# Improbable-AI/walk-these-ways

Hardware: AMD Instinct MI355X
Metric: env-steps/sec (sim+PPO) (higher is better)
Workload: dtype f32

## Files before the change

### include/go1ppo.h

```cpp
#ifndef GO1PPO_H
#define GO1PPO_H
#include <stdint.h>

#ifdef __cplusplus
extern "C" {
#endif

#define GO1PPO_ABI_VERSION 3
#define GO1PPO_MAX_ACTIONS 32

int go1ppo_elu_fwd(void* y, int64_t rows, int cols, int ld, const void* lat, int lat_ld, int npv, const void* wz,
                   int wz_ld, int lat_cols, void* stream);

int go1ppo_elu_bwd(const void* d, int ld_d, const void* h, int ld_h, int64_t rows, int cols, float* bias_grad, void* out,
                   int ld_out, void* stream);

typedef struct {
  const void* mean;
  const void* value;
  const float* std;
  int32_t head_ld, num_actions;
  int64_t rows;
  const int64_t* idx;
  const float* actions;
// ... 71 lines not shown
int go1ppo_store_step(const float* rewards, const uint8_t* dones, const uint8_t* time_outs, const int32_t* env_bins,
                      const float* values, float gamma, int64_t n, float* rewards_out, uint8_t* dones_out,
                      float* env_bins_out, void* stream);

int go1ppo_gae(const float* rewards, const uint8_t* dones, const float* values, const float* last_values, int T, int64_t N,
               float gamma, float lam, float* returns, float* advantages, double* stats, void* stream);

int go1ppo_normalize(float* adv, int64_t n, const double* stats, void* stream);


int go1ppo_ring_snapshot(const float* hist, int64_t ld_hist, int64_t N, int H, int no, void* ring, void* stream);

int go1ppo_ring_step(const float* obs, const float* priv, void* ring_dst, const void* ring_window, int64_t N, int H, int no,
                     int npv, int Kp, void* X, float* obs_store, float* priv_store, void* stream);

int go1ppo_ring_gather(const void* ring, const float* priv_store, const int64_t* idx, int64_t rows, int64_t N, int H, int no,
                       int npv, int Kp, void* X, void* stream);


int go1ppo_opt_partials(void);

int go1ppo_opt_prestep(const float* g, int64_t n, float gscale, float* partial, float* step, float* lr, const float* kl,
                       float kl_scale, float desired_kl, float lr_min, float lr_max, void* stream);

typedef struct {
  int64_t begin, count;
  const void* src;
  int64_t stride;
  int32_t kind, slabs, cols, zero_rows, zero_c0, zero_c1;
} Go1PpoGradPiece;
int go1ppo_grad_reduce(float* g, const Go1PpoGradPiece* device_pieces, int num_pieces, void* stream);
int go1ppo_opt_prestep_pieces(float* g, int64_t n, const Go1PpoGradPiece* device_pieces, int num_pieces, float gscale, float* partial,
                              float* step, float* lr, const float* kl, float kl_scale, float desired_kl, float lr_min, float lr_max,
                              void* stream);

#define GO1PPO_ADAM_MAX_TRANSPOSES 2
typedef struct {
  int32_t num_transposes, _pad;
  struct { int64_t start; int32_t rows, cols; void* dst; } transpose[GO1PPO_ADAM_MAX_TRANSPOSES];
} Go1PpoAdamExtras;
int go1ppo_opt_adam(float* p, float* g, float* m, float* v, int64_t start0, int64_t count0, int64_t start1,
                    int64_t count1, float gscale, const float* partial, float max_norm, const float* step, const float* lr,
                    float beta1, float beta2, float eps, void* body, int64_t n_body, float* tail, int64_t n_tail, int zero_grad,
                    float* zero_slot, const Go1PpoAdamExtras* extras, void* stream);

int go1ppo_sum_partials(const void* partials, int count, int64_t stride, int64_t rows, int cols, float* out, int zero_rows,
// ... 72 lines not shown
```

### walk-these-ways_amd/csrc/go1ppo.hip

```cpp
#include <hip/hip_runtime.h>
#include <stdint.h>
#include <string.h>
#include "../../include/go1ppo.h"

typedef uint16_t bf16_t;
static_assert(sizeof(Go1PpoAdamExtras) == 56 && sizeof(Go1PpoGemmArgs) == 96 && sizeof(Go1PpoWgradProblem) == 96 && sizeof(Go1PpoGradPiece) == 56, "ctypes mirrors (fused.py) assume these sizes");
typedef __attribute__((ext_vector_type(4))) float f32x4;

__device__ __forceinline__ float bf2f(bf16_t u) { return __uint_as_float(((uint32_t)u) << 16); }
__device__ __forceinline__ bf16_t f2bf(float f) {
  return __builtin_bit_cast(bf16_t, (__bf16)f);
}
struct alignas(16) Bf8 { bf16_t v[8]; };

typedef __attribute__((ext_vector_type(4))) uint32_t u32x4_t;
__device__ __forceinline__ void put16_wt(void* p, u32x4_t v) {
  asm volatile("global_store_dwordx4 %0, %1, off sc1\n\ts_nop 1" : : "v"((__attribute__((address_space(1))) void*)p), "v"(v) : "memory");
}
__device__ __forceinline__ void put16_wt(void* p, const Bf8& v) { put16_wt(p, __builtin_bit_cast(u32x4_t, v)); }
__device__ __forceinline__ void put16_wt(void* p, f32x4 v) { put16_wt(p, __builtin_bit_cast(u32x4_t, v)); }
__device__ __forceinline__ void put16_wt(void* p, uint4 v) { put16_wt(p, u32x4_t{v.x, v.y, v.z, v.w}); }

__device__ __forceinline__ float elu1(float x) {
  float em = x > -1e-3f ? fmaf(0.5f * x, x, x) : __expf(x) - 1.f;
// ... 522 lines not shown
  logp[r] = lp - (logs + A * HALF_LOG_2PI);
  values[r] = bf2f(value[r * head_ld]);
}

__global__ __launch_bounds__(256) void store_step_kernel(const float* rewards, const uint8_t* dones, const uint8_t* time_outs,
                                                         const int32_t* env_bins, const float* values, float gamma, int64_t n,
                                                         float* rewards_out, uint8_t* dones_out, float* env_bins_out) {
  int64_t i = (int64_t)blockIdx.x * 256 + threadIdx.x;
  if (i >= n) return;
  float r = rewards[i];
  if (time_outs) r += gamma * (values[i] * (time_outs[i] ? 1.f : 0.f));
  rewards_out[i] = r;
  dones_out[i] = dones[i];
  if (env_bins) env_bins_out[i] = (float)env_bins[i];
}

__global__ __launch_bounds__(256) void gae_kernel(const float* rewards, const uint8_t* dones, const float* values, const float* last_values,
                                                  int T, int64_t N, float gamma, float lam, float* returns, float* advantages, double* stats) {
  __shared__ double red[2][4];
  int64_t e = (int64_t)blockIdx.x * 256 + threadIdx.x;
  double s1 = 0.0, s2 = 0.0;
  if (e < N) {
    float adv = 0.f, next_v = last_values[e];
    for (int t = T - 1; t >= 0; t--) {
      const int64_t i = (int64_t)t * N + e;
      const float alive = 1.f - (float)dones[i];
      const float v = values[i];
      const float delta = rewards[i] + alive * gamma * next_v - v;
      adv = delta + alive * gamma * lam * adv;
      const float ret = adv + v;
// ... 18 lines not shown
  }
}

__global__ __launch_bounds__(256) void normalize_kernel(float* adv, int64_t n, const double* stats) {
  int64_t i = (int64_t)blockIdx.x * 256 + threadIdx.x;
  if (i >= n) return;
  const double cnt = stats[2], mean = stats[0] / cnt;
  double var = (stats[1] - cnt * mean * mean) / (cnt - 1.0);
  var = var > 0.0 ? var : 0.0;
  const float m = (float)mean, sd = (float)sqrt(var);
  adv[i] = (adv[i] - m) / (sd + 1e-8f);
}

#define OPT_BLOCKS 2048
template <bool NORM>
__device__ __forceinline__ float grad_pieces_pass(float* g, int64_t n, const Go1PpoGradPiece* __restrict__ pieces, int num_pieces, float gscale) {
  const int64_t tid = (int64_t)blockIdx.x * 256 + threadIdx.x, nth = (int64_t)gridDim.x * 256;
  auto gap_groups = [&](int64_t lo, int64_t hi) -> int64_t { return NORM && hi > lo ? (hi - lo + 7) >> 3 : 0; };
  auto piece_groups = [&](const Go1PpoGradPiece& P) -> int64_t { return P.kind == 0 ? gap_groups(P.begin, P.begin + P.count) : P.count >> 3; };
  int64_t total = 0;
  {
    int64_t cur = 0;
    for (int q = 0; q <= num_pieces; q++) {
      const int64_t pb = q < num_pieces ? pieces[q].begin : n;
      total += gap_groups(cur, pb < n ? pb : n);
      if (q == num_pieces) break;
      total += piece_groups(pieces[q]);
      cur = pieces[q].begin + pieces[q].count;
    }
  }
  float s = 0.f;
  auto plain8 = [&](int64_t i, int64_t hi) {
    if (i + 8 <= hi) {
      const f32x4 a = reinterpret_cast<const f32x4*>(g + i)[0] * gscale, b = reinterpret_cast<const f32x4*>(g + i)[1] * gscale;
#pragma unroll
      for (int e = 0; e < 4; e++) { s = fmaf(a[e], a[e], s); s = fmaf(b[e], b[e], s); }
    } else {
      for (int64_t j = i; j < hi; j++) { const float x = g[j] * gscale; s = fmaf(x, x, s); }
    }
  };
  for (int64_t f = tid; f < total; f += nth) {
    int64_t cum = 0, cur = 0;
    for (int q = 0; q <= num_pieces; q++) {
      const int64_t pb = q < num_pieces ? pieces[q].begin : n, ge = pb < n ? pb : n;
      const int64_t gg = gap_groups(cur, ge);
      if (f >= cum && f < cum + gg) plain8(cur + ((f - cum) << 3), ge);
      cum += gg;
      if (q == num_pieces) break;
      const Go1PpoGradPiece P = pieces[q];
      const int64_t pg = piece_groups(P);
      cur = P.begin + P.count;
      if (f >= cum && f < cum + pg) {
        const int64_t i = (f - cum) << 3;
        if (P.kind == 0) plain8(P.begin + i, cur);
        else {
          float acc[8] = {0.f, 0.f, 0.f, 0.f, 0.f, 0.f, 0.f, 0.f};
          if (P.kind == 1) {
            const float* src = (const float*)P.src + i;
            int b = 0;
            for (; b + 4 <= P.slabs; b += 4) {
              f32x4 lo[4], hi[4];
#pragma unroll
              for (int u = 0; u < 4; u++) {
                lo[u] = reinterpret_cast<const f32x4*>(src + (int64_t)(b + u) * P.stride)[0];
                hi[u] = reinterpret_cast<const f32x4*>(src + (int64_t)(b + u) * P.stride)[1];
              }
#pragma unroll
              for (int u = 0; u < 4; u++)
#pragma unroll
// ... 27 lines not shown
            const int c = (int)(i - row * P.cols);
            if (row < P.zero_rows && c < P.zero_c1 && c + 8 > P.zero_c0) {
#pragma unroll
              for (int e = 0; e < 8; e++)
                if (c + e >= P.zero_c0 && c + e < P.zero_c1) acc[e] = 0.f;
            }
          }
          float* out = g + P.begin + i;
          reinterpret_cast<f32x4*>(out)[0] = f32x4{acc[0], acc[1], acc[2], acc[3]};
          reinterpret_cast<f32x4*>(out)[1] = f32x4{acc[4], acc[5], acc[6], acc[7]};
          if (NORM) {
#pragma unroll
            for (int e = 0; e < 8; e++) { const float x = acc[e] * gscale; s = fmaf(x, x, s); }
          }
        }
      }
      cum += pg;
    }
  }
  return s;
}
__global__ __launch_bounds__(256) void grad_reduce_kernel(float* g, const Go1PpoGradPiece* __restrict__ pieces, int num_pieces) {
  grad_pieces_pass<false>(g, 0, pieces, num_pieces, 1.f);
}

__global__ __launch_bounds__(256) void prestep_kernel(const float* g, int64_t n, float gscale, float* partial, float* step, float* lr,
                                                      const float* kl, float kl_scale, float desired_kl, float lr_min, float lr_max,
                                                      const Go1PpoGradPiece* __restrict__ pieces, int num_pieces) {
  __shared__ float red[4];
  float s = 0.f;
  if (partial && pieces) {
    s = grad_pieces_pass<true>(const_cast<float*>(g), n, pieces, num_pieces, gscale);
// ... 60 lines not shown
        const int64_t ts = ex.transpose[t].start, te = ts + (int64_t)ex.transpose[t].rows * ex.transpose[t].cols;
        tr_chunk = tr_chunk || (j0 < count0) != (j1 < count0) || (i0 < te && i1 >= ts);
      }
    float gi[V], mi[V], vi[V], pi[V];
    if constexpr (V == 4) {
      const f32x4 g4 = *reinterpret_cast<const f32x4*>(g + i), m4 = *reinterpret_cast<const f32x4*>(m + i);
      const f32x4 v4 = *reinterpret_cast<const f32x4*>(v + i), p4 = *reinterpret_cast<const f32x4*>(p + i);
#pragma unroll
      for (int e = 0; e < 4; e++) { gi[e] = g4[e]; mi[e] = m4[e]; vi[e] = v4[e]; pi[e] = p4[e]; }
    } else {
      gi[0] = g[i]; mi[0] = m[i]; vi[0] = v[i]; pi[0] = p[i];
    }
#pragma unroll
    for (int e = 0; e < V; e++) {
      const float ge = gi[e] * gs;
      mi[e] = beta1 * mi[e] + (1.f - beta1) * ge;
      vi[e] = beta2 * vi[e] + (1.f - beta2) * ge * ge;
      pi[e] = pi[e] - step_size * mi[e] / (sqrtf(vi[e]) * inv_sqrt_bc2 + eps);
    }
    if constexpr (V == 4) {
      if (zero_grad) *reinterpret_cast<f32x4*>(g + i) = f32x4{0.f, 0.f, 0.f, 0.f};
      *reinterpret_cast<f32x4*>(m + i) = f32x4{mi[0], mi[1], mi[2], mi[3]};
      *reinterpret_cast<f32x4*>(v + i) = f32x4{vi[0], vi[1], vi[2], vi[3]};
      *reinterpret_cast<f32x4*>(p + i) = f32x4{pi[0], pi[1], pi[2], pi[3]};
    } else {
      if (zero_grad) g[i] = 0.f;
      m[i] = mi[0]; v[i] = vi[0]; p[i] = pi[0];
    }
    bf16_t pb[V];
#pragma unroll
    for (int e = 0; e < V; e++) pb[e] = f2bf(pi[e]);
    if (V == 4 && i + 4 <= n_body) {
      typedef __attribute__((ext_vector_type(4))) unsigned short us4_t;
// ... 303 lines not shown
    out[d] = ring_pack(e[0], e[1]);
  }
}

__global__ __launch_bounds__(256) void ring_snapshot_kernel(const float* __restrict__ hist, int64_t ld_hist, int64_t N, int H, int no,
                                                            uint32_t* __restrict__ ring) {
  const int nod = no >> 1;
  const int64_t total = N * H * nod, i = (int64_t)blockIdx.x * 256 + threadIdx.x;
  if (i >= total) return;
  const int c = (int)(i % nod);
  const int64_t r = i / nod, n = r % N, j = r / N;
  const float* src = hist + n * ld_hist + j * no + 2 * c;
  ring[(j * N + n) * nod + c] = ring_pack(src[0], src[1]);
}

__global__ __launch_bounds__(256) void ring_step_kernel(const float* __restrict__ obs, const float* __restrict__ priv, uint32_t* __restrict__ dst,
                                                        const uint32_t* __restrict__ window, int64_t N, int H, int no, int npv, int Kp,
                                                        uint32_t* __restrict__ X, float* __restrict__ obs_store, float* __restrict__ priv_store) {
  const int64_t n = (int64_t)blockIdx.x * 4 + (threadIdx.x >> 6);
  if (n >= N) return;
  const int lane = threadIdx.x & 63, nod = no >> 1;
  const float* o = obs + n * no;
  const float* pv = priv + n * npv;
  for (int c = lane; c < nod; c += 64) {
    if (dst) dst[n * nod + c] = ring_pack(o[2 * c], o[2 * c + 1]);
    if (obs_store) { obs_store[n * no + 2 * c] = o[2 * c]; obs_store[n * no + 2 * c + 1] = o[2 * c + 1]; }
  }
  if (priv_store)
    for (int c = lane; c < npv; c += 64) priv_store[n * npv + c] = pv[c];
  ring_row(window + n * nod, N * nod, o, pv, H, no, npv, Kp, X + n * (Kp >> 1));
}

__global__ __launch_bounds__(256) void ring_gather_kernel(const uint32_t* __restrict__ ring, const float* __restrict__ priv_store,
                                                          const int64_t* __restrict__ idx, int64_t rows, int64_t N, int H, int no, int npv,
                                                          int Kp, uint32_t* __restrict__ X) {
  const int64_t i = (int64_t)blockIdx.x * 4 + (threadIdx.x >> 6);
  if (i >= rows) return;
  const int64_t f = idx[i], s = f / N, n = f - s * N;
  const int nod = no >> 1;
  ring_row(ring + (s * N + n) * nod, N * nod, nullptr, priv_store + f * npv, H, no, npv, Kp, X + i * (Kp >> 1));
}

extern "C" int go1ppo_ring_snapshot(const float* hist, int64_t ld_hist, int64_t N, int H, int no, void* ring, void* stream) {
  if (!hist || !ring || N <= 0 || H <= 0 || no <= 0 || (no & 1) || ld_hist < (int64_t)H * no) return -1;
  const int64_t total = N * H * (no >> 1);
  ring_snapshot_kernel<<<dim3((unsigned)((total + 255) / 256)), dim3(256), 0, (hipStream_t)stream>>>(hist, ld_hist, N, H, no, (uint32_t*)ring);
  return hipGetLastError() == hipSuccess ? 0 : -9;
}

extern "C" int go1ppo_ring_step(const float* obs, const float* priv, void* ring_dst, const void* ring_window, int64_t N, int H, int no,
                                int npv, int Kp, void* X, float* obs_store, float* priv_store, void* stream) {
  if (!obs || !priv || !ring_window || !X || N <= 0 || H <= 0 || no <= 0 || (no & 1) || npv < 0 || npv > 256 || (Kp & 1) ||
      Kp < H * no + 1 + npv)
    return -1;
  ring_step_kernel<<<dim3((unsigned)((N + 3) / 4)), dim3(256), 0, (hipStream_t)stream>>>(obs, priv, (uint32_t*)ring_dst, (const uint32_t*)ring_window, N, H,
                                                                            no, npv, Kp, (uint32_t*)X, obs_store, priv_store);
  return hipGetLastError() == hipSuccess ? 0 : -9;
}

extern "C" int go1ppo_ring_gather(const void* ring, const float* priv_store, const int64_t* idx, int64_t rows, int64_t N, int H, int no,
                                  int npv, int Kp, void* X, void* stream) {
  if (!ring || !priv_store || !idx || !X || rows <= 0 || N <= 0 || H <= 0 || no <= 0 || (no & 1) || npv < 0 || (Kp & 1) ||
      Kp < H * no + 1 + npv)
    return -1;
  ring_gather_kernel<<<dim3((unsigned)((rows + 3) / 4)), dim3(256), 0, (hipStream_t)stream>>>((const uint32_t*)ring, priv_store, idx, rows, N,
                                                                                           H, no, npv, Kp, (uint32_t*)X);
  return hipGetLastError() == hipSuccess ? 0 : -9;
}

extern "C" int go1ppo_normalize(float* adv, int64_t n, const double* stats, void* stream) {
  if (!adv || !stats || n <= 0) return -1;
// ... 81 lines not shown

extern "C" int go1ppo_sum_partials(const void* partials, int count, int64_t stride, int64_t rows, int cols, float* out, int zero_rows,
                                   int zero_c0, int zero_c1, void* stream) {
  if (!partials || !out || count <= 0 || rows <= 0 || cols <= 0 || (cols & 7) || (stride & 7) || stride < rows * cols || !aligned16(partials) ||
      !aligned16(out) || zero_rows < 0 || zero_c0 < 0 || zero_c1 < zero_c0 || zero_c1 > cols)
    return -1;
  const int64_t total8 = rows * cols / 8;
  int64_t blocks = (total8 + 255) / 256;
  if (blocks > 4096) blocks = 4096;
  sum_partials_kernel<<<dim3((unsigned)blocks), dim3(256), 0, (hipStream_t)stream>>>((const bf16_t*)partials, count, stride, total8, cols, out,
                                                                                   zero_rows, zero_c0, zero_c1);
  return hipGetLastError() == hipSuccess ? 0 : -9;
}

extern "C" int go1ppo_opt_partials(void) { return OPT_BLOCKS; }

extern "C" int go1ppo_tail_fwd(const Go1PpoTailArgs* args, void* stream) {
  if (!args || args->num_nets <= 0 || args->num_nets > GO1PPO_TAIL_MAX_NETS) return -1;
  int64_t max_rows = 0;
  for (int i = 0; i < args->num_nets; i++) {
    const Go1PpoTailNet& N = args->net[i];
    if (!N.in || N.rows <= 0 || N.num_layers <= 0 || N.num_layers > GO1PPO_TAIL_MAX_LAYERS || (N.ld_in & 7) || !aligned16(N.in)) return -1;
    for (int l = 0; l < N.num_layers; l++) {
      const Go1PpoTailLayer& L = N.layer[l];
      if (!L.W || !L.bias || L.k_in <= 0 || L.k_in > TF_MAXK || (L.k_in & 31) || L.n_out <= 0 || L.n_out > TF_MAXK || (L.n_out & 15) ||
          !aligned16(L.W) || (l > 0 && L.k_in != N.layer[l - 1].n_out) || (L.out && L.ld_out < L.n_out))
        return -2;
    }
    if (N.rows > max_rows) max_rows = N.rows;
  }
// ... 32 lines not shown
```

### walk-these-ways_amd/go1_gym_learn/ppo_cse/fused.py

```python
import ctypes
import os

import torch

HEAD = 64
_HERE = os.path.dirname(os.path.abspath(__file__))
_LIB_PATH = os.path.normpath(os.path.join(_HERE, "..", "..", "csrc", "libgo1ppo.so"))
_lib = None


class Go1PpoLibraryMissing(RuntimeError):
    pass


class LossArgs(ctypes.Structure):
    _fields_ = [("mean", ctypes.c_void_p), ("value", ctypes.c_void_p), ("std", ctypes.c_void_p),
                ("head_ld", ctypes.c_int32), ("num_actions", ctypes.c_int32), ("rows", ctypes.c_int64),
                ("idx", ctypes.c_void_p), ("actions", ctypes.c_void_p), ("old_mu", ctypes.c_void_p),
                ("old_sigma", ctypes.c_void_p), ("old_logp", ctypes.c_void_p), ("advantages", ctypes.c_void_p),
                ("returns", ctypes.c_void_p), ("old_values", ctypes.c_void_p),
                ("clip_param", ctypes.c_float), ("value_loss_coef", ctypes.c_float), ("entropy_coef", ctypes.c_float),
                ("use_clipped_value_loss", ctypes.c_int32),
                ("d_mean", ctypes.c_void_p), ("d_value", ctypes.c_void_p), ("d_std", ctypes.c_void_p),
                ("d_mean_bias", ctypes.c_void_p), ("d_value_bias", ctypes.c_void_p), ("kl", ctypes.c_void_p),
# ... 57 lines not shown
class GemmArgs(ctypes.Structure):
    _fields_ = [("A", ctypes.c_void_p), ("B", ctypes.c_void_p), ("C", ctypes.c_void_p), ("bias", ctypes.c_void_p),
                ("H", ctypes.c_void_p)] + [(n, ctypes.c_int32) for n in
                                           ("M", "N", "K", "lda", "ldb", "ldc", "ldh", "epilogue", "elu_c0", "elu_c1", "elu_skip_c0", "elu_skip_c1", "bias_bf16", "_pad")]


class _AdamTranspose(ctypes.Structure):
    _fields_ = [("start", ctypes.c_int64), ("rows", ctypes.c_int32), ("cols", ctypes.c_int32), ("dst", ctypes.c_void_p)]


class AdamExtras(ctypes.Structure):
    _fields_ = [("num_transposes", ctypes.c_int32), ("_pad", ctypes.c_int32), ("transpose", _AdamTranspose * 2)]


EXPORTED_SYMBOLS = ["go1ppo_mlp2_fwd", "go1ppo_mlp2_bwd", "go1ppo_mlp2_tail_ppo", "go1ppo_mlp2_tail_mse", "go1ppo_gemm_nt", "go1ppo_gemm_nt_pair", "go1ppo_sum_partials", "go1ppo_wgrad_tn_plan", "go1ppo_wgrad_tn_batched", "go1ppo_tail_fwd", "go1ppo_elu_fwd", "go1ppo_elu_bwd", "go1ppo_loss", "go1ppo_mse", "go1ppo_wgrad", "go1ppo_wgrad_plan",
                    "go1ppo_wgrad_batched", "go1ppo_act",
                    "go1ppo_store_step", "go1ppo_ring_snapshot", "go1ppo_ring_step", "go1ppo_ring_gather", "go1ppo_gae", "go1ppo_normalize", "go1ppo_opt_partials", "go1ppo_opt_prestep",
                    "go1ppo_opt_prestep_pieces", "go1ppo_grad_reduce", "go1ppo_opt_adam", "go1ppo_version"]


def load_library(path=None):
    global _lib
    if _lib is not None and path is None:
        return _lib
    p = path or _LIB_PATH
    if not os.path.exists(p):
        raise Go1PpoLibraryMissing(f"{p} not found: run `python -c 'import __graft_entry__ as g; g.build()'` "
                                   "(hipcc --offload-arch=gfx950); the fused PPO update has no CPU fallback")
    L = ctypes.CDLL(p)
    vp, i32, i64 = ctypes.c_void_p, ctypes.c_int, ctypes.c_int64
    L.go1ppo_elu_fwd.argtypes = [vp, i64, i32, i32, vp, i32, i32, vp, i32, i32, vp]
    L.go1ppo_elu_bwd.argtypes = [vp, i32, vp, i32, i64, i32, vp, vp, i32, vp]
# ... 5 lines not shown
    L.go1ppo_gemm_nt.argtypes = [ctypes.POINTER(GemmArgs), vp]
    L.go1ppo_gemm_nt_pair.argtypes = [ctypes.POINTER(GemmArgs), ctypes.POINTER(GemmArgs), vp]
    L.go1ppo_sum_partials.argtypes = [vp, i32, i64, i64, i32, vp, i32, i32, i32, vp]
    L.go1ppo_mlp2_fwd.argtypes = [ctypes.POINTER(Mlp2Fwd), i32, vp]
    L.go1ppo_mlp2_bwd.argtypes = [ctypes.POINTER(Mlp2Bwd), i32, vp]
    L.go1ppo_mlp2_tail_ppo.argtypes = [ctypes.POINTER(Mlp2Tail), ctypes.POINTER(LossArgs), vp]
    L.go1ppo_mlp2_tail_mse.argtypes = [ctypes.POINTER(Mlp2Tail), ctypes.POINTER(MseArgs), vp]
    L.go1ppo_wgrad_batched.argtypes = [vp, i32, i32, vp]
    L.go1ppo_wgrad_tn_plan.argtypes = [ctypes.POINTER(WgradProblem), i32]
    L.go1ppo_wgrad_tn_batched.argtypes = [vp, i32, i32, vp]
    f32 = ctypes.c_float
    L.go1ppo_act.argtypes = [vp, vp, i32, vp, i32, i64, vp, vp, vp, vp, vp, vp, vp]
    L.go1ppo_store_step.argtypes = [vp, vp, vp, vp, vp, f32, i64, vp, vp, vp, vp]
    L.go1ppo_ring_snapshot.argtypes = [vp, i64, i64, i32, i32, vp, vp]
    L.go1ppo_ring_step.argtypes = [vp, vp, vp, vp, i64, i32, i32, i32, i32, vp, vp, vp, vp]
    L.go1ppo_ring_gather.argtypes = [vp, vp, vp, i64, i64, i32, i32, i32, i32, vp, vp]
    L.go1ppo_gae.argtypes = [vp, vp, vp, vp, i32, i64, f32, f32, vp, vp, vp, vp]
    L.go1ppo_normalize.argtypes = [vp, i64, vp, vp]
    L.go1ppo_opt_partials.argtypes = []
    L.go1ppo_opt_prestep.argtypes = [vp, i64, f32, vp, vp, vp, vp, f32, f32, f32, f32, vp]
    L.go1ppo_opt_prestep_pieces.argtypes = [vp, i64, vp, i32, f32, vp, vp, vp, vp, f32, f32, f32, f32, vp]
    L.go1ppo_grad_reduce.argtypes = [vp, vp, i32, vp]
    L.go1ppo_opt_adam.argtypes = [vp, vp, vp, vp, i64, i64, i64, i64, f32, vp, f32, vp, vp, f32, f32, f32, vp, i64, vp, i64, i32, vp,
                                  ctypes.POINTER(AdamExtras), vp]
    for name in EXPORTED_SYMBOLS[:-1]:
        getattr(L, name).restype = ctypes.c_int
    L.go1ppo_version.restype = ctypes.c_char_p
    if path is None:
        _lib = L
    return L


def _stream():
    return torch.cuda.current_stream().cuda_stream
# ... 524 lines not shown
            q.target, q.idx, q.num_train, q.npv, q.selective = target.data_ptr(), idx.data_ptr(), num_train, self.pol.npv, int(selective)
            q.d_pred_bias, q.train_loss, q.test_loss = self.G[f"adaptation.{last}.b"].data_ptr(), acc[2:].data_ptr(), acc[3:].data_ptr()
            _chk(self.lib.go1ppo_mlp2_tail_mse(arr, ctypes.byref(q), _stream()), "go1ppo_mlp2_tail_mse")
            return
        _chk(self.lib.go1ppo_mse(pred.data_ptr(), HEAD, target.data_ptr(), self.pol.npv, idx.data_ptr(), self.M, num_train,
                                 int(selective), dpred.data_ptr(), self.G[f"adaptation.{last}.b"].data_ptr(),
                                 acc[2:].data_ptr(), acc[3:].data_ptr(), _stream()), "go1ppo_mse")


def act(lib, mean, value, std, noise, st, s):
    _chk(lib.go1ppo_act(mean.data_ptr(), value.data_ptr(), _ld(mean), std.data_ptr(), std.numel(), mean.shape[0], noise.data_ptr(),
                        st.actions[s].data_ptr(), st.mu[s].data_ptr(), st.sigma[s].data_ptr(), st.values[s].data_ptr(),
                        st.actions_log_prob[s].data_ptr(), _stream()), "go1ppo_act")


def store_step(lib, st, s, rewards, dones, time_outs, env_bins, gamma):
    n = rewards.shape[0]
    for t, dt in ((rewards, torch.float32), (dones, torch.uint8)):
        assert t.is_contiguous() and t.dtype == dt and t.shape[0] == n
    if time_outs is not None:
        assert time_outs.is_contiguous() and time_outs.element_size() == 1
    if env_bins is not None:
        assert env_bins.is_contiguous() and env_bins.dtype == torch.int32
    _chk(lib.go1ppo_store_step(rewards.data_ptr(), dones.data_ptr(), _ptr(time_outs), _ptr(env_bins), st.values[s].data_ptr(), gamma, n,
                               st.rewards[s].data_ptr(), st.dones[s].data_ptr(), st.env_bins[s].data_ptr() if env_bins is not None else None,
                               _stream()), "go1ppo_store_step")


def ring_step(lib, st, s, obs, privileged_obs, obs_history, X):
    N, no, H = st.num_envs, st.obs_ring.shape[2], st.history_length
    npv = st.privileged_observations.shape[-1]
    for t in (obs, privileged_obs):
        assert t.dtype == torch.float32 and t.is_contiguous() and t.shape[0] == N
    assert X.dtype == torch.bfloat16 and X.is_contiguous() and tuple(X.shape) == (N, st.padded_width)
    if s == 0:
        assert obs_history.dtype == torch.float32 and obs_history.stride(1) == 1 and tuple(obs_history.shape) == (N, H * no)
        _chk(lib.go1ppo_ring_snapshot(obs_history.data_ptr(), obs_history.stride(0), N, H, no, st.obs_ring.data_ptr(), _stream()),
             "go1ppo_ring_snapshot")
    dst = None if s == 0 else st.obs_ring[s + H - 1].data_ptr()
    _chk(lib.go1ppo_ring_step(obs.data_ptr(), privileged_obs.data_ptr(), dst, st.obs_ring[s].data_ptr(), N, H, no, npv, st.padded_width,
                              X.data_ptr(), st.observations[s].data_ptr(), st.privileged_observations[s].data_ptr(), _stream()),
         "go1ppo_ring_step")


def ring_gather(lib, st, idx, X):
    N, no, H = st.num_envs, st.obs_ring.shape[2], st.history_length
    priv = st.privileged_observations
    assert idx.dtype == torch.int64 and idx.is_contiguous() and X.is_contiguous() and tuple(X.shape) == (idx.numel(), st.padded_width)
    assert priv.dtype == torch.float32 and priv.is_contiguous()
    _chk(lib.go1ppo_ring_gather(st.obs_ring.data_ptr(), priv.data_ptr(), idx.data_ptr(), idx.numel(), N, H, no, priv.shape[-1],
                                st.padded_width, X.data_ptr(), _stream()), "go1ppo_ring_gather")


def gae(lib, st, last_values, gamma, lam, stats):
    T, N = st.num_transitions_per_env, st.num_envs
    stats.zero_()
    _chk(lib.go1ppo_gae(st.rewards.data_ptr(), st.dones.data_ptr(), st.values.data_ptr(), last_values.data_ptr(), T, N, gamma, lam,
# ... 58 lines not shown
```

### walk-these-ways_amd/go1_gym_learn/ppo_cse/ppo.py

```python
import math
import os
import sys

import torch
import torch.distributed as dist
import torch.nn.functional as F
import torch.optim as optim
from params_proto import PrefixProto

from go1_gym_learn.ppo_cse import ActorCritic
from go1_gym_learn.ppo_cse import RolloutStorage
from go1_gym_learn.ppo_cse import caches
from go1_gym_learn.ppo_cse.flat_policy import FlatPolicy


class PPO_Args(PrefixProto):
    value_loss_coef = 1.0
    use_clipped_value_loss = True
    clip_param = 0.2
    entropy_coef = 0.01
    num_learning_epochs = 5
    num_mini_batches = 4
    learning_rate = 1.e-3
    adaptation_module_learning_rate = 1.e-3
# ... 94 lines not shown
        self.std = torch.zeros(self.n_std, device=device).requires_grad_()
        kw = dict(fused=True, capturable=True) if self.on_gpu else {}
        self._acc = torch.zeros(4, device=device)
        self._idx_all, self._graphs, self._updates_done = None, {}, 0
        self._collectives_capturable = None
        self._pregathered, self._Xall = False, None
        lr = torch.tensor(PPO_Args.learning_rate, device=device) if self.on_gpu else PPO_Args.learning_rate
        self.optimizer = optim.Adam([self.master], lr=lr, **kw)
        self.adaptation_module_optimizer = optim.Adam([self.master], lr=PPO_Args.adaptation_module_learning_rate, **kw)
        self.transition = RolloutStorage.Transition()
        self._lr = torch.tensor(PPO_Args.learning_rate, device=device)
        self.dp = bool(PPO_Args.data_parallel and (_world() > 1 or (_force_dp() and dist.is_available() and dist.is_initialized())))
        self.fused = bool(self.bf16 and PPO_Args.use_fused_kernels and self.policy.act is torch.nn.ELU)
        self._roll_net = self._train_net = None
        self._roll_noise = None
        self._update_graph_ok = True
        self._opt = self._opt_ad = None
        if self.on_gpu and PPO_Args.use_tuned_gemms:
            _enable_tuned_gemms()
        self._ad_grad_views = [self.master.grad]
        if self.fused:
            from go1_gym_learn.ppo_cse import fused
            self._fused_lib = fused.load_library()
            pol, ns = self.policy, self.n_std
            self._opt = fused.FusedAdam(self._fused_lib, self.master, self.body, self.std, n, PPO_Args.learning_rate, ranges=[(0, n + ns)])
            self._opt_ad = fused.FusedAdam(self._fused_lib, self.master, self.body, self.std, n, PPO_Args.adaptation_module_learning_rate,
                                           ranges=[(0, pol.adaptation_numel)])
            self._lr = self._opt.lr
            self._ad_grad_views = [self.master.grad[:pol.adaptation_numel]]
        if self.dp:
# ... 72 lines not shown
        self._X_roll = torch.zeros_like(self._last_hist) if ring else None
        if self.fused:
            from go1_gym_learn.ppo_cse.fused import FusedNet
            self._roll_net = FusedNet(self.policy, self.body, None, num_envs, self._fused_lib, with_grad=False, two_streams=False)

    def test_mode(self):
        self.actor_critic.test()

    def train_mode(self):
        self.actor_critic.train()

    def act(self, obs, privileged_obs, obs_history):
        t = self.transition
        if self.storage.ring:
            return self._act_ring(obs, privileged_obs, obs_history)
        slot = self.storage.observation_histories[self.storage.step]
        self.storage.write_history(slot, obs_history, privileged_obs)
        t.observation_histories = slot
        if self._roll_net is not None and slot.shape[0] == self._roll_net.M:
            return self._act_fused(slot, obs, privileged_obs)
        mean, value = self._infer(slot)
        std = self.std.detach()
        t.actions = mean + std * torch.randn_like(mean)
        t.values = value.detach()
        t.actions_log_prob = gaussian_log_prob(t.actions, mean, std)
        t.action_mean = mean
        t.action_sigma = std.expand_as(mean)
        self._snapshot_obs(obs, privileged_obs)
        return t.actions

# ... 3 lines not shown
        if s >= st.num_transitions_per_env:
            raise AssertionError("Rollout buffer overflow")
        st.observations[s].copy_(obs)
        st.privileged_observations[s].copy_(privileged_obs)
        t.observations = t.critic_observations = st.observations[s]
        t.privileged_observations = st.privileged_observations[s]

    def _act_ring(self, obs, privileged_obs, obs_history):
        from go1_gym_learn.ppo_cse import fused
        st = self.storage
        s = st.step
        if s >= st.num_transitions_per_env:
            raise AssertionError("Rollout buffer overflow")
        if st.num_envs != self._roll_net.M:
            raise AssertionError("ring storage needs the static-buffer inference engine of its own batch size")
        fused.ring_step(self._fused_lib, st, s, obs.contiguous(), privileged_obs.contiguous(), obs_history, self._X_roll)
        self.transition.observation_histories = self._X_roll
        return self._act_fused(self._X_roll, obs, privileged_obs, stored=True)

    def _act_fused(self, slot, obs, privileged_obs, stored=False):
        from go1_gym_learn.ppo_cse import fused
        t, st = self.transition, self.storage
        s = st.step
        if s >= st.num_transitions_per_env:
            raise AssertionError("Rollout buffer overflow")
        with torch.no_grad():
            mean, value, _ = self._roll_net.forward(slot)
            T = st.num_transitions_per_env
            if s == 0 or self._roll_noise is None or tuple(self._roll_noise.shape) != (T, slot.shape[0], self.n_std):
                self._roll_noise = torch.randn(T, slot.shape[0], self.n_std, device=slot.device)
            noise = self._roll_noise[s]
# ... 24 lines not shown
        t.env_bins = infos["env_bins"]
        if 'time_outs' in infos:
            t.rewards += PPO_Args.gamma * torch.squeeze(t.values * infos['time_outs'].unsqueeze(1).to(self.device), 1)
        self.storage.add_transitions(t)
        t.clear()
        self.actor_critic.reset(dones)

    def _process_env_step_fused(self, rewards, dones, infos):
        from go1_gym_learn.ppo_cse import fused
        t, st = self.transition, self.storage
        s = st.step
        tos = infos['time_outs'] if 'time_outs' in infos else None
        if tos is not None and tos.dtype == torch.bool:
            tos = tos.view(torch.uint8)
        bins = infos["env_bins"][:rewards.shape[0]]
        fused.store_step(self._fused_lib, st, s, rewards.contiguous(), dones if dones.dtype == torch.uint8 else dones.to(torch.uint8), tos,
                         bins if bins.dtype == torch.int32 else bins.to(torch.int32), PPO_Args.gamma)
        st.step += 1
        t.clear()
        self.actor_critic.reset(dones)

    def compute_returns(self, last_critic_obs, last_critic_privileged_obs):
        self.storage.write_history(self._last_hist, last_critic_obs, last_critic_privileged_obs)
        _, last_values = self._infer(self._last_hist)
        self.storage.compute_returns(last_values.clone(), PPO_Args.gamma, PPO_Args.lam,
                                     fused_lib=self._fused_lib if self.fused else None)

    def _adapt_lr(self, kl_mean):
        lr = self._lr
        dk = PPO_Args.desired_kl
        down = torch.clamp(lr / 1.5, min=1e-5)
        up = torch.clamp(lr * 1.5, max=1e-2)
        new = torch.where(kl_mean > dk * 2.0, down, torch.where((kl_mean < dk / 2.0) & (kl_mean > 0.0), up, lr))
        self._lr.copy_(new)
        for group in self.optimizer.param_groups:
            if torch.is_tensor(group['lr']):
                group['lr'].copy_(new)
# ... 320 lines not shown
```

Before: 5.303 million.

## Defer store_step into next ring_step kernel and LDS-index gradient pieces

Each env step's reward/done/bin store is no longer its own kernel launch. It is deferred and fused into the following ring_step kernel, with one lane per environment doing the store. The gradient-norm pieces pass now copies piece descriptors into shared memory, prefix-sums the segment offsets with a wave scan, and binary-searches them per element group instead of linearly walking all pieces. Adam updates are rewritten with explicit fmaf. The deferred store adds bookkeeping risk: it must be flushed before returns are computed or on a non-ring path.

Result: no change. 5.343 million, median of 6 (+0.8%).

```diff
diff --git a/include/go1ppo.h b/include/go1ppo.h
--- a/include/go1ppo.h
+++ b/include/go1ppo.h
@@ -109,6 +109,11 @@
 int go1ppo_ring_step(const float* obs, const float* priv, void* ring_dst, const void* ring_window, int64_t N, int H, int no,
                      int npv, int Kp, void* X, float* obs_store, float* priv_store, void* stream);
 
+int go1ppo_ring_store_step(const float* obs, const float* priv, void* ring_dst, const void* ring_window, int64_t N, int H, int no,
+                           int npv, int Kp, void* X, float* obs_store, float* priv_store, const float* rewards,
+                           const uint8_t* dones, const uint8_t* time_outs, const int32_t* env_bins, const float* values, float gamma,
+                           float* rewards_out, uint8_t* dones_out, float* env_bins_out, void* stream);
+
 int go1ppo_ring_gather(const void* ring, const float* priv_store, const int64_t* idx, int64_t rows, int64_t N, int H, int no,
                        int npv, int Kp, void* X, void* stream);
 
@@ -125,6 +130,7 @@
   int32_t kind, slabs, cols, zero_rows, zero_c0, zero_c1;
 } Go1PpoGradPiece;
 int go1ppo_grad_reduce(float* g, const Go1PpoGradPiece* device_pieces, int num_pieces, void* stream);
+int go1ppo_opt_lds_pieces(void);
 int go1ppo_opt_prestep_pieces(float* g, int64_t n, const Go1PpoGradPiece* device_pieces, int num_pieces, float gscale, float* partial,
                               float* step, float* lr, const float* kl, float kl_scale, float desired_kl, float lr_min, float lr_max,
                               void* stream);
diff --git a/walk-these-ways_amd/csrc/go1ppo.hip b/walk-these-ways_amd/csrc/go1ppo.hip
--- a/walk-these-ways_amd/csrc/go1ppo.hip
+++ b/walk-these-ways_amd/csrc/go1ppo.hip
@@ -560,6 +560,24 @@
   dones_out[i] = dones[i];
   if (env_bins) env_bins_out[i] = (float)env_bins[i];
 }
+struct StoreStepArgs {
+  const float* rewards; const uint8_t* dones; const uint8_t* time_outs; const int32_t* env_bins; const float* values; float gamma;
+  float* rewards_out; uint8_t* dones_out; float* env_bins_out;
+};
+struct StoreStepVals { float r, bin; uint8_t d; };
+__device__ __forceinline__ StoreStepVals store_step_load(const StoreStepArgs& S, int64_t i) {
+  StoreStepVals v;
+  v.r = S.rewards[i];
+  if (S.time_outs) v.r = __builtin_fmaf(S.gamma, S.values[i] * (S.time_outs[i] ? 1.f : 0.f), v.r);
+  v.d = S.dones[i];
+  v.bin = S.env_bins ? (float)S.env_bins[i] : 0.f;
+  return v;
+}
+__device__ __forceinline__ void store_step_put(const StoreStepArgs& S, int64_t i, const StoreStepVals& v) {
+  S.rewards_out[i] = v.r;
+  S.dones_out[i] = v.d;
+  if (S.env_bins) S.env_bins_out[i] = v.bin;
+}
 
 __global__ __launch_bounds__(256) void gae_kernel(const float* rewards, const uint8_t* dones, const float* values, const float* last_values,
                                                   int T, int64_t N, float gamma, float lam, float* returns, float* advantages, double* stats) {
@@ -608,45 +626,21 @@
 
 #define OPT_BLOCKS 2048
 template <bool NORM>
-__device__ __forceinline__ float grad_pieces_pass(float* g, int64_t n, const Go1PpoGradPiece* __restrict__ pieces, int num_pieces, float gscale) {
-  const int64_t tid = (int64_t)blockIdx.x * 256 + threadIdx.x, nth = (int64_t)gridDim.x * 256;
-  auto gap_groups = [&](int64_t lo, int64_t hi) -> int64_t { return NORM && hi > lo ? (hi - lo + 7) >> 3 : 0; };
-  auto piece_groups = [&](const Go1PpoGradPiece& P) -> int64_t { return P.kind == 0 ? gap_groups(P.begin, P.begin + P.count) : P.count >> 3; };
-  int64_t total = 0;
-  {
-    int64_t cur = 0;
-    for (int q = 0; q <= num_pieces; q++) {
-      const int64_t pb = q < num_pieces ? pieces[q].begin : n;
-      total += gap_groups(cur, pb < n ? pb : n);
-      if (q == num_pieces) break;
-      total += piece_groups(pieces[q]);
-      cur = pieces[q].begin + pieces[q].count;
-    }
-  }
-  float s = 0.f;
-  auto plain8 = [&](int64_t i, int64_t hi) {
-    if (i + 8 <= hi) {
-      const f32x4 a = reinterpret_cast<const f32x4*>(g + i)[0] * gscale, b = reinterpret_cast<const f32x4*>(g + i)[1] * gscale;
-#pragma unroll
-      for (int e = 0; e < 4; e++) { s = fmaf(a[e], a[e], s); s = fmaf(b[e], b[e], s); }
-    } else {
-      for (int64_t j = i; j < hi; j++) { const float x = g[j] * gscale; s = fmaf(x, x, s); }
-    }
-  };
-  for (int64_t f = tid; f < total; f += nth) {
-    int64_t cum = 0, cur = 0;
-    for (int q = 0; q <= num_pieces; q++) {
-      const int64_t pb = q < num_pieces ? pieces[q].begin : n, ge = pb < n ? pb : n;
-      const int64_t gg = gap_groups(cur, ge);
-      if (f >= cum && f < cum + gg) plain8(cur + ((f - cum) << 3), ge);
-      cum += gg;
-      if (q == num_pieces) break;
-      const Go1PpoGradPiece P = pieces[q];
-      const int64_t pg = piece_groups(P);
-      cur = P.begin + P.count;
-      if (f >= cum && f < cum + pg) {
-        const int64_t i = (f - cum) << 3;
-        if (P.kind == 0) plain8(P.begin + i, cur);
+__device__ __forceinline__ int64_t gp_gap_groups(int64_t lo, int64_t hi) { return NORM && hi > lo ? (hi - lo + 7) >> 3 : 0; }
+template <bool NORM>
+__device__ __forceinline__ int64_t gp_piece_groups(const Go1PpoGradPiece& P) { return P.kind == 0 ? gp_gap_groups<NORM>(P.begin, P.begin + P.count) : P.count >> 3; }
+__device__ __forceinline__ void gp_plain8(const float* g, int64_t i, int64_t hi, float gscale, float& s) {
+  if (i + 8 <= hi) {
+    const f32x4 a = reinterpret_cast<const f32x4*>(g + i)[0] * gscale, b = reinterpret_cast<const f32x4*>(g + i)[1] * gscale;
+#pragma unroll
+    for (int e = 0; e < 4; e++) { s = fmaf(a[e], a[e], s); s = fmaf(b[e], b[e], s); }
+  } else {
+    for (int64_t j = i; j < hi; j++) { const float x = g[j] * gscale; s = fmaf(x, x, s); }
+  }
+}
+template <bool NORM>
+__device__ __forceinline__ void gp_piece8(float* g, const Go1PpoGradPiece& P, int64_t i, float gscale, float& s) {
+        if (P.kind == 0) gp_plain8(g, P.begin + i, P.begin + P.count, gscale, s);
         else {
           float acc[8] = {0.f, 0.f, 0.f, 0.f, 0.f, 0.f, 0.f, 0.f};
           if (P.kind == 1) {
@@ -704,8 +698,79 @@
             for (int e = 0; e < 8; e++) { const float x = acc[e] * gscale; s = fmaf(x, x, s); }
           }
         }
-      }
+}
+template <bool NORM>
+__device__ __forceinline__ float grad_pieces_pass_walk(float* g, int64_t n, const Go1PpoGradPiece* __restrict__ pieces, int num_pieces, float gscale) {
+  const int64_t tid = (int64_t)blockIdx.x * 256 + threadIdx.x, nth = (int64_t)gridDim.x * 256;
+  int64_t total = 0;
+  {
+    int64_t cur = 0;
+    for (int q = 0; q <= num_pieces; q++) {
+      const int64_t pb = q < num_pieces ? pieces[q].begin : n;
+      total += gp_gap_groups<NORM>(cur, pb < n ? pb : n);
+      if (q == num_pieces) break;
+      total += gp_piece_groups<NORM>(pieces[q]);
+      cur = pieces[q].begin + pieces[q].count;
+    }
+  }
+  float s = 0.f;
+  for (int64_t f = tid; f < total; f += nth) {
+    int64_t cum = 0, cur = 0;
+    for (int q = 0; q <= num_pieces; q++) {
+      const int64_t pb = q < num_pieces ? pieces[q].begin : n, ge = pb < n ? pb : n;
+      const int64_t gg = gp_gap_groups<NORM>(cur, ge);
+      if (f >= cum && f < cum + gg) gp_plain8(g, cur + ((f - cum) << 3), ge, gscale, s);
+      cum += gg;
+      if (q == num_pieces) break;
+      const Go1PpoGradPiece P = pieces[q];
+      const int64_t pg = gp_piece_groups<NORM>(P);
+      cur = P.begin + P.count;
+      if (f >= cum && f < cum + pg) gp_piece8<NORM>(g, P, (f - cum) << 3, gscale, s);
       cum += pg;
+    }
+  }
+  return s;
+}
+#define GP_LDS_PIECES 63
+template <bool NORM>
+__device__ __forceinline__ float grad_pieces_pass(float* g, int64_t n, const Go1PpoGradPiece* __restrict__ pieces, int num_pieces, float gscale) {
+  if (num_pieces > GP_LDS_PIECES) return grad_pieces_pass_walk<NORM>(g, n, pieces, num_pieces, gscale);
+  static_assert(sizeof(Go1PpoGradPiece) == 56, "the cooperative load copies 7 x 8 bytes per piece");
+  __shared__ __attribute__((aligned(16))) Go1PpoGradPiece sp[GP_LDS_PIECES];
+  __shared__ int64_t cum[2 * GP_LDS_PIECES + 2];
+  for (int w = threadIdx.x; w < num_pieces * 7; w += 256) reinterpret_cast<uint64_t*>(sp)[w] = reinterpret_cast<const uint64_t*>(pieces)[w];
+  __syncthreads();
+  auto gap_lo = [&](int q) -> int64_t { return q ? sp[q - 1].begin + sp[q - 1].count : 0; };
+  auto gap_hi = [&](int q) -> int64_t { const int64_t pb = q < num_pieces ? sp[q].begin : n; return pb < n ? pb : n; };
+  if (threadIdx.x < 64) {
+    const int q = threadIdx.x;
+    int64_t gg = 0, pg = 0;
+    if (q <= num_pieces) gg = gp_gap_groups<NORM>(gap_lo(q), gap_hi(q));
+    if (q < num_pieces) pg = gp_piece_groups<NORM>(sp[q]);
+    long long incl = gg + pg;
+    for (int o = 1; o < 64; o <<= 1) {
+      const long long up = __shfl_up(incl, o, 64);
+      if (q >= o) incl += up;
+    }
+    if (q <= num_pieces) { cum[2 * q] = incl - pg - gg; cum[2 * q + 1] = incl - pg; }
+  }
+  __syncthreads();
+  const int nseg = 2 * num_pieces + 1;
+  const int64_t total = cum[nseg];
+  const int64_t tid = (int64_t)blockIdx.x * 256 + threadIdx.x, nth = (int64_t)gridDim.x * 256;
+  float s = 0.f;
+  for (int64_t f = tid; f < total; f += nth) {
+    int seg = 0;
+#pragma unroll
+    for (int step = 64; step > 0; step >>= 1)
+      if (seg + step < nseg && cum[seg + step] <= f) seg += step;
+    const int q = seg >> 1;
+    const int64_t i = (f - cum[seg]) << 3;
+    if (seg & 1) {
+      const Go1PpoGradPiece P = sp[q];
+      gp_piece8<NORM>(g, P, i, gscale, s);
+    } else {
+      gp_plain8(g, gap_lo(q) + i, gap_hi(q), gscale, s);
     }
   }
   return s;
@@ -796,9 +861,9 @@
 #pragma unroll
     for (int e = 0; e < V; e++) {
       const float ge = gi[e] * gs;
-      mi[e] = beta1 * mi[e] + (1.f - beta1) * ge;
-      vi[e] = beta2 * vi[e] + (1.f - beta2) * ge * ge;
-      pi[e] = pi[e] - step_size * mi[e] / (sqrtf(vi[e]) * inv_sqrt_bc2 + eps);
+      mi[e] = __builtin_fmaf(beta1, mi[e], (1.f - beta1) * ge);
+      vi[e] = __builtin_fmaf(beta2, vi[e], ((1.f - beta2) * ge) * ge);
+      pi[e] = pi[e] - (step_size * mi[e]) / __builtin_fmaf(sqrtf(vi[e]), inv_sqrt_bc2, eps);
     }
     if constexpr (V == 4) {
       if (zero_grad) *reinterpret_cast<f32x4*>(g + i) = f32x4{0.f, 0.f, 0.f, 0.f};
@@ -1132,11 +1197,9 @@
   ring[(j * N + n) * nod + c] = ring_pack(src[0], src[1]);
 }
 
-__global__ __launch_bounds__(256) void ring_step_kernel(const float* __restrict__ obs, const float* __restrict__ priv, uint32_t* __restrict__ dst,
-                                                        const uint32_t* __restrict__ window, int64_t N, int H, int no, int npv, int Kp,
-                                                        uint32_t* __restrict__ X, float* __restrict__ obs_store, float* __restrict__ priv_store) {
-  const int64_t n = (int64_t)blockIdx.x * 4 + (threadIdx.x >> 6);
-  if (n >= N) return;
+__device__ __forceinline__ void ring_step_env(int64_t n, const float* __restrict__ obs, const float* __restrict__ priv, uint32_t* __restrict__ dst,
+                                              const uint32_t* __restrict__ window, int64_t N, int H, int no, int npv, int Kp,
+                                              uint32_t* __restrict__ X, float* __restrict__ obs_store, float* __restrict__ priv_store) {
   const int lane = threadIdx.x & 63, nod = no >> 1;
   const float* o = obs + n * no;
   const float* pv = priv + n * npv;
@@ -1147,6 +1210,26 @@
   if (priv_store)
     for (int c = lane; c < npv; c += 64) priv_store[n * npv + c] = pv[c];
   ring_row(window + n * nod, N * nod, o, pv, H, no, npv, Kp, X + n * (Kp >> 1));
+}
+__global__ __launch_bounds__(256) void ring_step_kernel(const float* __restrict__ obs, const float* __restrict__ priv, uint32_t* __restrict__ dst,
+                                                        const uint32_t* __restrict__ window, int64_t N, int H, int no, int npv, int Kp,
+                                                        uint32_t* __restrict__ X, float* __restrict__ obs_store, float* __restrict__ priv_store) {
+  const int64_t n = (int64_t)blockIdx.x * 4 + (threadIdx.x >> 6);
+  if (n >= N) return;
+  ring_step_env(n, obs, priv, dst, window, N, H, no, npv, Kp, X, obs_store, priv_store);
+}
+
+__global__ __launch_bounds__(256) void ring_store_step_kernel(const float* __restrict__ obs, const float* __restrict__ priv, uint32_t* __restrict__ dst,
+                                                              const uint32_t* __restrict__ window, int64_t N, int H, int no, int npv, int Kp,
+                                                              uint32_t* __restrict__ X, float* __restrict__ obs_store, float* __restrict__ priv_store,
+                                                              StoreStepArgs S) {
+  const int64_t n = (int64_t)blockIdx.x * 4 + (threadIdx.x >> 6);
+  if (n >= N) return;
+  const bool storer = (threadIdx.x & 63) == 63;
+  StoreStepVals v = {0.f, 0.f, 0};
+  if (storer) v = store_step_load(S, n);
+  ring_step_env(n, obs, priv, dst, window, N, H, no, npv, Kp, X, obs_store, priv_store);
+  if (storer) store_step_put(S, n, v);
 }
 
 __global__ __launch_bounds__(256) void ring_gather_kernel(const uint32_t* __restrict__ ring, const float* __restrict__ priv_store,
@@ -1173,6 +1256,20 @@
     return -1;
   ring_step_kernel<<<dim3((unsigned)((N + 3) / 4)), dim3(256), 0, (hipStream_t)stream>>>(obs, priv, (uint32_t*)ring_dst, (const uint32_t*)ring_window, N, H,
                                                                             no, npv, Kp, (uint32_t*)X, obs_store, priv_store);
+  return hipGetLastError() == hipSuccess ? 0 : -9;
+}
+
+extern "C" int go1ppo_ring_store_step(const float* obs, const float* priv, void* ring_dst, const void* ring_window, int64_t N, int H, int no,
+                                      int npv, int Kp, void* X, float* obs_store, float* priv_store, const float* rewards,
+                                      const uint8_t* dones, const uint8_t* time_outs, const int32_t* env_bins, const float* values,
+                                      float gamma, float* rewards_out, uint8_t* dones_out, float* env_bins_out, void* stream) {
+  if (!obs || !priv || !ring_window || !X || N <= 0 || H <= 0 || no <= 0 || (no & 1) || npv < 0 || npv > 256 || (Kp & 1) ||
+      Kp < H * no + 1 + npv)
+    return -1;
+  if (!rewards || !dones || !values || !rewards_out || !dones_out || (env_bins && !env_bins_out)) return -1;
+  const StoreStepArgs S = {rewards, dones, time_outs, env_bins, values, gamma, rewards_out, dones_out, env_bins_out};
+  ring_store_step_kernel<<<dim3((unsigned)((N + 3) / 4)), dim3(256), 0, (hipStream_t)stream>>>(
+      obs, priv, (uint32_t*)ring_dst, (const uint32_t*)ring_window, N, H, no, npv, Kp, (uint32_t*)X, obs_store, priv_store, S);
   return hipGetLastError() == hipSuccess ? 0 : -9;
 }
 
@@ -1284,6 +1381,7 @@
 }
 
 extern "C" int go1ppo_opt_partials(void) { return OPT_BLOCKS; }
+extern "C" int go1ppo_opt_lds_pieces(void) { return GP_LDS_PIECES; }
 
 extern "C" int go1ppo_tail_fwd(const Go1PpoTailArgs* args, void* stream) {
   if (!args || args->num_nets <= 0 || args->num_nets > GO1PPO_TAIL_MAX_NETS) return -1;
diff --git a/walk-these-ways_amd/go1_gym_learn/ppo_cse/fused.py b/walk-these-ways_amd/go1_gym_learn/ppo_cse/fused.py
--- a/walk-these-ways_amd/go1_gym_learn/ppo_cse/fused.py
+++ b/walk-these-ways_amd/go1_gym_learn/ppo_cse/fused.py
@@ -95,8 +95,8 @@
 
 
 EXPORTED_SYMBOLS = ["go1ppo_mlp2_fwd", "go1ppo_mlp2_bwd", "go1ppo_mlp2_tail_ppo", "go1ppo_mlp2_tail_mse", "go1ppo_gemm_nt", "go1ppo_gemm_nt_pair", "go1ppo_sum_partials", "go1ppo_wgrad_tn_plan", "go1ppo_wgrad_tn_batched", "go1ppo_tail_fwd", "go1ppo_elu_fwd", "go1ppo_elu_bwd", "go1ppo_loss", "go1ppo_mse", "go1ppo_wgrad", "go1ppo_wgrad_plan",
-                    "go1ppo_wgrad_batched", "go1ppo_act",
-                    "go1ppo_store_step", "go1ppo_ring_snapshot", "go1ppo_ring_step", "go1ppo_ring_gather", "go1ppo_gae", "go1ppo_normalize", "go1ppo_opt_partials", "go1ppo_opt_prestep",
+                    "go1ppo_wgrad_batched", "go1ppo_act", "go1ppo_ring_store_step",
+                    "go1ppo_store_step", "go1ppo_ring_snapshot", "go1ppo_ring_step", "go1ppo_ring_gather", "go1ppo_gae", "go1ppo_normalize", "go1ppo_opt_partials", "go1ppo_opt_lds_pieces", "go1ppo_opt_prestep",
                     "go1ppo_opt_prestep_pieces", "go1ppo_grad_reduce", "go1ppo_opt_adam", "go1ppo_version"]
 
 
@@ -132,10 +132,12 @@
     L.go1ppo_store_step.argtypes = [vp, vp, vp, vp, vp, f32, i64, vp, vp, vp, vp]
     L.go1ppo_ring_snapshot.argtypes = [vp, i64, i64, i32, i32, vp, vp]
     L.go1ppo_ring_step.argtypes = [vp, vp, vp, vp, i64, i32, i32, i32, i32, vp, vp, vp, vp]
+    L.go1ppo_ring_store_step.argtypes = [vp, vp, vp, vp, i64, i32, i32, i32, i32, vp, vp, vp, vp, vp, vp, vp, vp, f32, vp, vp, vp, vp]
     L.go1ppo_ring_gather.argtypes = [vp, vp, vp, i64, i64, i32, i32, i32, i32, vp, vp]
     L.go1ppo_gae.argtypes = [vp, vp, vp, vp, i32, i64, f32, f32, vp, vp, vp, vp]
     L.go1ppo_normalize.argtypes = [vp, i64, vp, vp]
     L.go1ppo_opt_partials.argtypes = []
+    L.go1ppo_opt_lds_pieces.argtypes = []
     L.go1ppo_opt_prestep.argtypes = [vp, i64, f32, vp, vp, vp, vp, f32, f32, f32, f32, vp]
     L.go1ppo_opt_prestep_pieces.argtypes = [vp, i64, vp, i32, f32, vp, vp, vp, vp, f32, f32, f32, f32, vp]
     L.go1ppo_grad_reduce.argtypes = [vp, vp, i32, vp]
@@ -690,7 +692,7 @@
                         st.actions_log_prob[s].data_ptr(), _stream()), "go1ppo_act")
 
 
-def store_step(lib, st, s, rewards, dones, time_outs, env_bins, gamma):
+def _store_step_args(st, s, rewards, dones, time_outs, env_bins, gamma):
     n = rewards.shape[0]
     for t, dt in ((rewards, torch.float32), (dones, torch.uint8)):
         assert t.is_contiguous() and t.dtype == dt and t.shape[0] == n
@@ -698,12 +700,16 @@
         assert time_outs.is_contiguous() and time_outs.element_size() == 1
     if env_bins is not None:
         assert env_bins.is_contiguous() and env_bins.dtype == torch.int32
-    _chk(lib.go1ppo_store_step(rewards.data_ptr(), dones.data_ptr(), _ptr(time_outs), _ptr(env_bins), st.values[s].data_ptr(), gamma, n,
-                               st.rewards[s].data_ptr(), st.dones[s].data_ptr(), st.env_bins[s].data_ptr() if env_bins is not None else None,
-                               _stream()), "go1ppo_store_step")
-
-
-def ring_step(lib, st, s, obs, privileged_obs, obs_history, X):
+    return n, (rewards.data_ptr(), dones.data_ptr(), _ptr(time_outs), _ptr(env_bins), st.values[s].data_ptr(), gamma), \
+        (st.rewards[s].data_ptr(), st.dones[s].data_ptr(), st.env_bins[s].data_ptr() if env_bins is not None else None)
+
+
+def store_step(lib, st, s, rewards, dones, time_outs, env_bins, gamma):
+    n, ins, outs = _store_step_args(st, s, rewards, dones, time_outs, env_bins, gamma)
+    _chk(lib.go1ppo_store_step(*ins, n, *outs, _stream()), "go1ppo_store_step")
+
+
+def ring_step(lib, st, s, obs, privileged_obs, obs_history, X, store=None):
     N, no, H = st.num_envs, st.obs_ring.shape[2], st.history_length
     npv = st.privileged_observations.shape[-1]
     for t in (obs, privileged_obs):
@@ -714,9 +720,14 @@
         _chk(lib.go1ppo_ring_snapshot(obs_history.data_ptr(), obs_history.stride(0), N, H, no, st.obs_ring.data_ptr(), _stream()),
              "go1ppo_ring_snapshot")
     dst = None if s == 0 else st.obs_ring[s + H - 1].data_ptr()
-    _chk(lib.go1ppo_ring_step(obs.data_ptr(), privileged_obs.data_ptr(), dst, st.obs_ring[s].data_ptr(), N, H, no, npv, st.padded_width,
-                              X.data_ptr(), st.observations[s].data_ptr(), st.privileged_observations[s].data_ptr(), _stream()),
-         "go1ppo_ring_step")
+    ring = (obs.data_ptr(), privileged_obs.data_ptr(), dst, st.obs_ring[s].data_ptr(), N, H, no, npv, st.padded_width,
+            X.data_ptr(), st.observations[s].data_ptr(), st.privileged_observations[s].data_ptr())
+    if store is not None:
+        n, ins, outs = _store_step_args(st, *store)
+        assert n == N
+        _chk(lib.go1ppo_ring_store_step(*ring, *ins, *outs, _stream()), "go1ppo_ring_store_step")
+        return
+    _chk(lib.go1ppo_ring_step(*ring, _stream()), "go1ppo_ring_step")
 
 
 def ring_gather(lib, st, idx, X):
diff --git a/walk-these-ways_amd/go1_gym_learn/ppo_cse/ppo.py b/walk-these-ways_amd/go1_gym_learn/ppo_cse/ppo.py
--- a/walk-these-ways_amd/go1_gym_learn/ppo_cse/ppo.py
+++ b/walk-these-ways_amd/go1_gym_learn/ppo_cse/ppo.py
@@ -132,6 +132,7 @@
         self.fused = bool(self.bf16 and PPO_Args.use_fused_kernels and self.policy.act is torch.nn.ELU)
         self._roll_net = self._train_net = None
         self._roll_noise = None
+        self._owed_store = None
         self._update_graph_ok = True
         self._opt = self._opt_ad = None
         if self.on_gpu and PPO_Args.use_tuned_gemms:
@@ -234,6 +235,7 @@
         t = self.transition
         if self.storage.ring:
             return self._act_ring(obs, privileged_obs, obs_history)
+        self._flush_store()
         slot = self.storage.observation_histories[self.storage.step]
         self.storage.write_history(slot, obs_history, privileged_obs)
         t.observation_histories = slot
@@ -267,7 +269,12 @@
             raise AssertionError("Rollout buffer overflow")
         if st.num_envs != self._roll_net.M:
             raise AssertionError("ring storage needs the static-buffer inference engine of its own batch size")
-        fused.ring_step(self._fused_lib, st, s, obs.contiguous(), privileged_obs.contiguous(), obs_history, self._X_roll)
+        owed = self._owed_store
+        if owed is not None and owed[0] != s - 1:
+            self._flush_store()
+            owed = None
+        self._owed_store = None
+        fused.ring_step(self._fused_lib, st, s, obs.contiguous(), privileged_obs.contiguous(), obs_history, self._X_roll, store=owed)
         self.transition.observation_histories = self._X_roll
         return self._act_fused(self._X_roll, obs, privileged_obs, stored=True)
 
@@ -322,13 +329,24 @@
         if tos is not None and tos.dtype == torch.bool:
             tos = tos.view(torch.uint8)
         bins = infos["env_bins"][:rewards.shape[0]]
-        fused.store_step(self._fused_lib, st, s, rewards.contiguous(), dones if dones.dtype == torch.uint8 else dones.to(torch.uint8), tos,
-                         bins if bins.dtype == torch.int32 else bins.to(torch.int32), PPO_Args.gamma)
+        store = (s, rewards.contiguous(), dones if dones.dtype == torch.uint8 else dones.to(torch.uint8), tos,
+                 bins if bins.dtype == torch.int32 else bins.to(torch.int32), PPO_Args.gamma)
+        if st.ring and s + 1 < st.num_transitions_per_env:
+            self._owed_store = store
+        else:
+            fused.store_step(self._fused_lib, st, *store)
         st.step += 1
         t.clear()
         self.actor_critic.reset(dones)
 
+    def _flush_store(self):
+        if self._owed_store is not None:
+            from go1_gym_learn.ppo_cse import fused
+            owed, self._owed_store = self._owed_store, None
+            fused.store_step(self._fused_lib, self.storage, *owed)
+
     def compute_returns(self, last_critic_obs, last_critic_privileged_obs):
+        self._flush_store()
         self.storage.write_history(self._last_hist, last_critic_obs, last_critic_privileged_obs)
         _, last_values = self._infer(self._last_hist)
         self.storage.compute_returns(last_values.clone(), PPO_Args.gamma, PPO_Args.lam,
```
